# nihalsid/retrieval-fuse

Measured on AMD Instinct MI355X. Metric: 64^3 TSDF chunks/sec (retrieve+attend+refine), higher is better.
Workload: dtype f32

## Files before the change

### include/rfuse.h

```cpp
#ifndef RFUSE_H
#define RFUSE_H

#include <stdint.h>
#include <stddef.h>

#ifdef __cplusplus
extern "C" {
#endif

#define RF_OK 0
#define RF_E_INVALID (-1)
#define RF_E_UNSUPPORTED (-2)
#define RF_E_LAUNCH (-3)
#define RF_E_WORKSPACE (-4)

int rf_abi_version(void);
const char* rf_last_error(void);


int rf_conv3_pack_weight(const float* w_oidhw, int cout, int cin, float* w_packed, void* stream);
size_t rf_conv3_packed_floats(int cout, int cin);

int rf_gn_stats(const float* src0, int c0, const float* src1, int c1, int n, int edge,
                const float* gamma, const float* beta, int groups, float eps,
                float* gn_affine, void* ws, size_t ws_bytes, void* stream);
size_t rf_gn_stats_ws_bytes(int n, int groups);

int rf_conv3d_k3_gn_relu(const float* src0, int c0, const float* src1, int c1, int n, int edge,
                         const float* gn_affine, const float* w_packed, int cout,
                         float* out, void* stream);

int rf_conv3d_k3_gn_relu_stats(const float* src0, int c0, const float* src1, int c1, int n, int edge,
                               const float* gn_affine, const float* w_packed, int cout,
                               float* out, double* stats, void* stream);
int rf_conv3d_stats_tiles(int c0, int c1, int n, int edge, int cout);

int rf_gn_from_stats(const double* stats0, int c0, int tiles0, const double* stats1, int c1, int tiles1, int n, int edge,
                     const float* gamma, const float* beta, int groups, float eps, float* gn_affine, void* stream);

int rf_conv3d_k3_gn_relu_direct(const float* src0, int c0, const float* src1, int c1, int n, int edge,
                                const float* gn_affine, const float* w_oidhw, int cout,
                                float* out, void* stream);

int rf_maxpool3d_2(const float* x, int n, int c, int edge, float* out, void* stream);
int rf_maxpool3d_2_stats(const float* x, int n, int c, int edge, float* out, double* stats, void* stream);
int rf_maxpool_stats_tiles(int edge);

int rf_conv1x1_tanh(const float* x, int n, int c, size_t voxels, const float* w, const float* b,
                    float post_add, float post_mul, float* out, void* stream);

int rf_conv3d_valid_leaky(const float* x, int n, int cin, int s, const float* w, const float* bias, int cout, int k,
                          int stride, float slope, float* out, void* stream);

int rf_conv3d_valid_leaky_mfma(const float* x, int n, int cin, int s, const float* w_packed, const float* bias, int cout, int k,
                               int stride, float slope, float* out, void* stream);
int rf_convv_pack_weight(const float* w_oidhw, int cout, int cin, int k, float* w_packed, void* stream);
size_t rf_convv_packed_floats(int cout, int cin, int k);

int rf_conv3d_valid_lds_supported(int n, int cin, int s, int cout, int k, int stride);
int rf_conv3d_valid_leaky_lds(const float* x, int n, int cin, int s, const float* w_packed, const float* bias, int cout, int k,
                              int stride, float slope, float* out, void* stream);
int rf_convv_lds_pack_weight(const float* w_oidhw, int cout, int cin, int k, float* w_packed, void* stream);
size_t rf_convv_lds_packed_floats(int cout, int cin, int k);

int rf_conv3d_valid_split_supported(int n, int cin, int s, int cout, int k, int stride);
int rf_conv3d_valid_leaky_split(const float* x, int n, int cin, int s, const void* w_packed, const float* bias, int cout, int k,
                                int stride, float slope, float* out, void* stream);
int rf_conv3d_valid_leaky_split_ex(const void* x, int in_split, int n, int cin, int s, const void* w_packed, const float* bias, int cout, int k,
                                   int stride, float slope, void* out, int out_split, void* stream);
int rf_convv_split_pack_weight(const float* w_oidhw, int cout, int cin, int k, int s, int stride, void* w_packed, void* stream);
size_t rf_convv_split_packed_bytes(int cout, int cin, int k, int s, int stride);
int rf_conv3d_valid_split_pg_supported(int n, int cin, int s, int cout, int k, int stride);
int rf_conv3d_valid_leaky_split_pg(const void* x, int n, int cin, int s, const void* w_packed, const float* bias, int cout, int k, int stride,
                                   float slope, void* out, void* stream);
int rf_convv_split_pg_pack_weight(const float* w_oidhw, int cout, int cin, int k, int s, int stride, void* w_packed, void* stream);
size_t rf_convv_split_pg_packed_bytes(int cout, int cin, int k, int s, int stride);

int rf_conv3d_valid_valu_supported(int n, int cin, int s, int cout, int k, int stride);
int rf_conv3d_valid_leaky_valu(const float* x, int n, int cin, int s, const float* w_t, const float* bias, int cout, int k,
                               int stride, float slope, float* out, void* stream);
int rf_conv3d_valid_leaky_valu_ex(const float* x, int n, int cin, int s, const float* w_t, const float* bias, int cout, int k,
                                  int stride, float slope, void* out, int out_split, void* stream);

int rf_conv3d_pool_supported(int c0, int c1, int n, int edge, int cout);
int rf_conv3d_k3_gn_relu_pool(const float* src0, int c0, const float* src1, int c1, int n, int edge,
                              const float* gn_affine, const float* w_packed, int cout,
                              float* out, double* stats, float* pool_out, double* pool_stats, void* stream);

size_t rf_conv3_up_packed_floats(int cout, int c0, int c1);
int rf_conv3_up_pack_weight(const float* w_oidhw, int cout, int c0, int c1, float* w_packed, void* stream);
int rf_conv3d_up_supported(int c0, int c1, int n, int edge, int cout);
int rf_conv3d_up_stats_tiles(int c0, int c1, int n, int edge, int cout);
int rf_conv3d_up_variant(int c0, int c1, int n, int edge, int cout);
int rf_conv3d_up_k3_gn_relu(const float* src0, int c0, const float* src1, int c1, int n, int edge,
                            const float* gn_affine, const float* w_packed, int cout, float* out, double* stats, void* stream);

size_t rf_conv3_up_split_packed_bytes(int cout, int c0, int c1);
int rf_conv3_up_split_pack_weight(const float* w_oidhw, int cout, int c0, int c1, void* w_packed, void* stream);
int rf_conv3d_up_split_supported(int c0, int c1, int n, int edge, int cout);
int rf_conv3d_up_split_stats_tiles(int c0, int c1, int n, int edge, int cout);
int rf_conv3d_up_split_k3_gn_relu(const float* src0, int c0, const float* src1, int c1, int n, int edge,
                                  const float* gn_affine, const void* w_packed, int cout, float* out, double* stats, void* stream);

size_t rf_conv3_split_packed_bytes(int cout, int cin);
int rf_conv3_split_pack_weight(const float* w_oidhw, int cout, int cin, void* w_packed, void* stream);
int rf_conv3d_split_supported(int c0, int c1, int n, int edge, int cout);
int rf_conv3d_split_k3_gn_relu(const float* src, int cin, int n, int edge, const float* gn_affine, const void* w_packed, int cout,
                               float* out, double* stats, float* pool_out, double* pool_stats, void* stream);

size_t rf_conv3_e2_split_packed_bytes(int cout, int cin, int edge);
int rf_conv3_e2_split_pack_weight(const float* w_oidhw, int cout, int cin, int edge, void* w_packed, void* stream);
int rf_conv3d_e2_split_supported(int cin, int n, int edge, int cout);
int rf_conv3d_e2_split_k3_gn_relu(const float* src, int cin, int n, int edge, const float* gn_affine, const void* w_packed, int cout,
                                  float* out, double* stats, void* stream);

size_t rf_split_act_bytes(int n, int c, int edge);
int rf_conv3d_cin1_presplit_supported(int n, int edge, int cout, int next_groups);
int rf_conv3d_cin1_presplit(const float* src, int n, int edge, const float* in_gamma, const float* in_beta, float in_eps, const float* w_packed, int cout,
                            const float* next_gamma, const float* next_beta, int next_groups, float eps, void* out_presplit, void* stream);

int rf_conv3d_split_pointwise_supported(int cin, int n, int edge, int cout);
int rf_conv3d_split_k3_gn_relu_pointwise_tanh(const float* src, int cin, int n, int edge, const float* gn_affine, const void* w_packed, int cout,
                                              const float* pw_w, const float* pw_b, float post_add, float post_mul, float* out1, void* stream);

int rf_conv3d_split_presplit_supported(int cin, int n, int edge, int cout, int next_groups);
int rf_conv3d_split_presplit(const float* src, int cin, int n, int edge, const float* gn_affine, const void* w_packed, int cout, const float* next_gamma,
                             const float* next_beta, int next_groups, float eps, void* out_presplit, double* stats, void* stream);
int rf_conv3d_up_split_presplit_supported(int c0, int c1, int n, int edge, int cout, int next_groups);
int rf_conv3d_up_split_presplit(const float* src0, int c0, const float* src1, int c1, int n, int edge, const float* gn_affine, const void* w_packed,
                                int cout, const float* next_gamma, const float* next_beta, int next_groups, float eps, void* out_presplit,
                                double* stats, void* stream);
int rf_conv3d_split_pre_supported(int cin, int n, int edge, int cout);
int rf_conv3d_split_pre_stats_tiles(int cin, int n, int edge, int cout);
int rf_conv3d_split_pre_k3_relu(const void* src_presplit, int cin, int n, int edge, const void* w_packed, int cout,
                                float* out, double* stats, float* pool_out, double* pool_stats, void* stream);
int rf_conv3d_up_split_presplit_pm_supported(int c0, int c1, int n, int edge, int cout, int next_groups);
int rf_conv3d_up_split_presplit_pm(const float* src0, int c0, const float* src1, int c1, int n, int edge, const float* gn_affine, const void* w_packed,
                                   int cout, const float* next_gamma, const float* next_beta, int next_groups, float eps, void* out_presplit_pm,
                                   double* stats, void* stream);
int rf_conv3d_split_pre_pm_supported(int cin, int n, int edge, int cout);
int rf_conv3d_split_pre_pm_k3_relu(const void* src_presplit_pm, int cin, int n, int edge, const void* w_packed, int cout,
                                   float* out, double* stats, float* pool_out, double* pool_stats, void* stream);


int rf_conv3d_k3_gn(const float* src0, int c0, const float* src1, int c1, int n, int edge,
                    const float* gn_affine, const float* w_packed, int cout, int relu, float* out, void* stream);
int rf_relu_backward(const float* dy, const float* y, size_t count, float* out, void* stream);
int rf_relu_backward_amax_slots(void);
int rf_relu_backward_amax(const float* dy, const float* y, size_t count, float* out, float* amax_slots, void* stream);
int rf_dgrad_scale_affine(const float* amax_slots, int rows, float* affine, float* scales, void* stream);
int rf_conv3d_split_k3_gn_supported(int cin, int n, int edge, int cout);
int rf_conv3d_split_k3_gn(const float* src, int cin, int n, int edge, const float* gn_affine, const void* w_packed, int cout, int relu,
                          float* out, void* stream);
int rf_maxpool3d_2_backward(const float* x, const float* dy, int n, int c, int edge, float* dx, void* stream);
int rf_upsample3d_2(const float* lo, int n, int c, int edge_lo, float* hi, void* stream);
int rf_sumpool3d_2(const float* hi, int n, int c, int edge, float* lo, void* stream);
int rf_gn_backward(const float* x, const float* dxn, int n, int c, int edge, const float* gamma, int groups, float eps, const float* dxn_inv_scale,
                   float* dx, float* dgamma, float* dbeta, void* ws, size_t ws_bytes, void* stream);
size_t rf_gn_backward_ws_bytes(int n, int c, int edge);
int rf_conv3d_k3_wgrad(const float* x, int cin, int n, int edge, const float* gn_affine, const float* dz, int cout, float* dw, void* ws,
                       size_t ws_bytes, void* stream);
size_t rf_conv3d_k3_wgrad_ws_bytes(int cin, int cout, int n, int edge);
int rf_conv3d_k3_wgrad_split_supported(int cin, int cout, int n, int edge);
size_t rf_conv3d_k3_wgrad_split_ws_bytes(int cin, int cout, int n, int edge);
int rf_conv3d_k3_wgrad_split(const float* x, int cin, int n, int edge, const float* gn_affine, const float* dz, int cout, const float* scales,
                             float* dw, void* ws, size_t ws_bytes, void* stream);

size_t rf_conv3d_valid_leaky_backward_ws_bytes(int n, int cout, int so);
int rf_conv3d_valid_leaky_backward(const float* dy, const float* y, int n, int cout, int so, float slope, float* dz, float* db, void* ws,
                                   size_t ws_bytes, void* stream);
size_t rf_convv_dgrad_packed_floats(int cout, int cin, int k);
int rf_conv3d_valid_dgrad(const float* dz, int n, int cout, int so, const float* wd_packed, int cin, int k, int stride, int s, float* dx, void* stream);
size_t rf_conv3d_valid_wgrad_ws_bytes(int n, int cin, int cout, int so, int k);
int rf_conv3d_valid_wgrad(const float* x, int n, int cin, int s, const float* dz, int cout, int k, int stride, float* dw, void* ws, size_t ws_bytes,
                          void* stream);


int rf_unfold3d(const float* x, int b, int c, int s, int e, float* rows, void* stream);
int rf_fold3d(const float* rows, int b, int c, int s, int e, float* x, void* stream);


int rf_linear_pack_weight(const float* w, int nout, int nin, float* w_packed, void* stream);
size_t rf_linear_packed_floats(int nout, int nin);

#define RF_ACT_NONE 0
#define RF_ACT_RELU 1
#define RF_ACT_LEAKY 2
int rf_linear(const float* x, int rows, int nin, const float* w_packed, const float* bias, int nout,
              int act, float slope, float* y, void* stream);

int rf_linear_wgrad(const float* a, const float* b, int K, int M, int N, float* dw, void* ws, size_t ws_bytes, void* stream);
size_t rf_linear_wgrad_ws_bytes(int K, int M, int N);

int rf_l2_normalize_rows(float* x, int rows, int dim, float eps, void* stream);


#define RF_ATTN_SOFTMAX 0
#define RF_ATTN_GUMBEL_HARD 1
int rf_attn_fuse(const float* x, const float* p, const float* xf, const float* pf, const float* noise,
                 int b, int k, int d, int f, int mode, float sharpness,
                 float* out, float* scores_out, float* weights_out, void* stream);

int rf_attn_gather_retrieved(const float* src, int src_layout, int b, int k, int c, int s, int e, int t,
                             float* p_rows, void* stream);

size_t rf_attn_mlp_split_packed_floats(int n_in);
int rf_attn_mlp_split_pack(const float* w1, const float* w2, const float* w3, const float* w4, int n_in, float* packed_split, void* stream);
int rf_attn_mlp_split_rows(const float* x, int rows, int n_in, const float* packed, const float* packed_split, float* out, void* stream);
int rf_attn_mlp_split_volume(const float* src, int b, int kv, int c, int s, int t, const float* packed, const float* packed_split,
                             float* out, void* stream);
size_t rf_attn_mlp_packed_floats(int n_in);
int rf_attn_mlp_pack(const float* w1, const float* b1, const float* w2, const float* b2, const float* w3, const float* b3,
                     const float* w4, const float* b4, int n_in, float* packed, void* stream);
int rf_attn_mlp_rows(const float* x, int rows, int n_in, const float* packed, float* out, void* stream);
int rf_attn_mlp_volume(const float* src, int b, int kv, int c, int s, int t, const float* packed, float* out, void* stream);
int rf_attn_weights(const float* xf, const float* pf, const float* noise, int rows, int k, int f, int mode, float sharpness,
                    float* weights, float* switches, float* scores_out, void* stream);
int rf_attn_weights_sampled(const float* xf, const float* pf, int rows, int k, int f, float sharpness, void* rng_state,
                            float* weights, float* switches, float* scores_out, float* noise_out, void* stream);
int rf_attn_blend(const float* x, const float* retrieved, int b, int k, int c, int s, int t, const float* weights,
                  const float* switches, float* out, void* stream);


int rf_query_windows(const float* raw, int b, int s, int ps, int ctx, float pad_value, float mean, float stddev,
                     float* out, void* stream);

int rf_gather_windows(const float* grid, int n, int c, int g, int w, int step, int np, float* out, void* stream);
int rf_gather_windows_split(const void* grid, int n, int c, int g, int w, int step, int np, void* out, void* stream);

int rf_db_pack_embeddings(const float* emb, int64_t n, int dim, float* packed, void* stream);
size_t rf_db_packed_floats(int64_t n, int dim);

int rf_l2_topk(const float* q, int nq, int dim, const float* db_packed, int64_t n, int64_t row_base, int k2, int algo,
               float* out_dist, int64_t* out_idx, void* ws, size_t ws_bytes, void* stream);
size_t rf_l2_topk_ws_bytes(int nq, int64_t n, int k2);
int rf_l2_topk_keys(const float* q, int nq, int dim, const float* db_packed, int64_t n, int64_t row_base, int k2, int algo,
                    uint64_t* out_keys, void* ws, size_t ws_bytes, void* stream);
int rf_topk_merge_keys(const uint64_t* in_keys, int parts, int nq, int k2, float* out_dist, int64_t* out_idx, void* stream);

int rf_topk_merge(const float* in_dist, const int64_t* in_idx, int parts, int nq, int k2,
                  float* out_dist, int64_t* out_idx, void* stream);

int rf_demote_same_scene(const float* dist, const int64_t* idx, int nq, int k2, const int32_t* db_meta,
                         const int32_t* query_scene, const uint8_t* query_keep, int K, int32_t* out_meta, float* out_dist,
                         int64_t* out_idx, void* stream);

int rf_gather_patches(const float* db_volumes, int64_t n_scenes, const int32_t* meta, int chunks, int K,
                      float trunc_fill, float trunc_ratio, float mean, float stddev, int layout,
                      float* out, void* stream);

int rf_gather_patches_f16(const void* db_volumes_f16, int64_t n_scenes, const int32_t* meta, int chunks, int K,
                          float trunc_fill, float trunc_ratio, float mean, float stddev, int layout,
                          float* out, void* stream);
int rf_compose_overlap(const void* db_volumes, int half, int64_t n_scenes, const float* mapping, const int32_t* boxes, int P, int K, int sx, int sy, int sz,
                       float trunc_fill, float trunc_ratio, float* out, float* dist_ws, void* stream);

int rf_gather_rows(const float* src, int64_t n_src, const int64_t* idx, int64_t m, int width, float* out, void* stream);


size_t rf_conv3d_split_pre_pool_presplit_scratch_floats(int cout);
int rf_conv3d_split_pre_pool_presplit_supported(int cin, int n, int edge, int cout, int next_groups);
int rf_conv3d_split_pre_k3_relu_pool_presplit(const void* src_presplit, int cin, int n, int edge, const void* w_packed, int cout, float* pool_scratch,
                                              double* pool_stats, const float* next_gamma, const float* next_beta, int next_groups, float eps,
                                              void* out_presplit, void* stream);
int rf_conv3d_split_pre_presplit_supported(int cin, int n, int edge, int cout, int next_groups);
int rf_conv3d_split_pre_presplit(const void* src_presplit, int cin, int n, int edge, const void* w_packed, int cout, const float* next_gamma,
                                 const float* next_beta, int next_groups, float eps, void* out_presplit, double* stats, void* stream);
// ... 30 lines not shown
```

### retrieval-fuse_amd/csrc/conv3d_e2_split.hip

```cpp
#include "common.h"
#include "split_operand.h"

namespace {
constexpr int E2_NC = 256;
constexpr int E2_STEP_H8 = (E2_NC / 16) * 2 * 64;
constexpr int E2_LDS_BYTES = 2 * E2_STEP_H8 * 16;
}

__host__ __device__ static inline size_t e2_chunks(int cout, int edge) { return ((size_t)cout * (edge == 2 ? 8 : 1) + E2_NC - 1) / E2_NC; }
__host__ __device__ static inline size_t e2_ksteps(int cin, int edge) { return edge == 2 ? (size_t)(cin + 3) / 4 : (size_t)(cin + 31) / 32; }

extern "C" size_t rf_conv3_e2_split_packed_bytes(int cout, int cin, int edge) {
    return e2_chunks(cout, edge) * e2_ksteps(cin, edge) * E2_STEP_H8 * 16;
}

__global__ void k_conv3_e2_split_pack(const float* __restrict__ w, int cout, int cin, int edge, h8* __restrict__ wp, size_t total) {
    const int ksteps = (int)e2_ksteps(cin, edge);
    for (size_t i = (size_t)blockIdx.x * blockDim.x + threadIdx.x; i < total; i += (size_t)gridDim.x * blockDim.x) {
        const int lane = (int)(i & 63), piece = (int)((i >> 6) & 1), t = (int)((i >> 7) & 15);
        const size_t st = i >> 11;
        const int s = (int)(st % ksteps), chunk = (int)(st / ksteps);
        const int col = chunk * E2_NC + t * 16 + (lane & 15);
        h8 out;
#pragma unroll
// ... 8 lines not shown
            } else {
                const int co = col, ci = 32 * s + 8 * (lane >> 4) + u;
                if (co < cout && ci < cin) val = (double)w[((size_t)co * cin + ci) * 27 + 13];
            }
            _Float16 h, l;
            rf_split_weight(val, h, l);
            out[u] = piece == 0 ? h : l;
        }
        wp[i] = out;
    }
}

extern "C" int rf_conv3_e2_split_pack_weight(const float* w_oidhw, int cout, int cin, int edge, void* w_packed, void* stream) {
    RF_REQUIRE(w_oidhw && w_packed && cout > 0 && cin > 0 && (edge == 1 || edge == 2), RF_E_INVALID, "rf_conv3_e2_split_pack_weight: bad arguments");
    const size_t total = rf_conv3_e2_split_packed_bytes(cout, cin, edge) / 16;
    return rf_launch<k_conv3_e2_split_pack>("rf_conv3_e2_split_pack_weight", dim3(rf_blocks(total, 256, 4096)), dim3(256), (hipStream_t)stream, w_oidhw, cout, cin, edge,
                                            reinterpret_cast<h8*>(w_packed), total);
}

struct E2Args {
    const float* src;
    const float4* affine;
    const h8* wp;
    float* out;
    double2* stats;
    int cin, cout, n;
};

template <int V, int MT>
__global__ __launch_bounds__(256, 2) void k_conv3_e2_split(E2Args a) {
    constexpr int WN = MT == 64 ? 2 : 4, NJ = 16 / WN;
    extern __shared__ __attribute__((aligned(16))) unsigned char lds_raw[];
    h8* bufs = reinterpret_cast<h8*>(lds_raw);
    const int tid = threadIdx.x, lane = tid & 63;
    const int wave = __builtin_amdgcn_readfirstlane(tid >> 6);
    const int wm = MT == 64 ? wave >> 1 : 0, wn = MT == 64 ? wave & 1 : wave;
    const int li = lane & 15, kg = lane >> 4;
    const int n0 = blockIdx.x * MT, chunk = blockIdx.y;
    const int cin = a.cin, cout = a.cout, ksteps = V == 8 ? cin >> 2 : (cin + 31) >> 5;
    const h8* __restrict__ wsrc = a.wp + (size_t)chunk * ksteps * E2_STEP_H8 + tid;

    const float* xrow[2];
    const float4* arow[2];
#pragma unroll
    for (int i = 0; i < 2; ++i) {
        int sm = n0 + (2 * wm + i) * 16 + li;
        sm = sm < a.n ? sm : a.n - 1;
        xrow[i] = a.src + (V == 8 ? ((size_t)sm * cin + kg) * 8 : (size_t)sm * cin + kg * 8);
        arow[i] = a.affine + (V == 8 ? (size_t)sm * cin + kg : (size_t)sm * cin + kg * 8);
    }
    f32x4 hi[2][NJ], lo[2][NJ];
#pragma unroll
    for (int i = 0; i < 2; ++i)
#pragma unroll
        for (int j = 0; j < NJ; ++j) { hi[i][j] = f32x4{0.f, 0.f, 0.f, 0.f}; lo[i][j] = f32x4{0.f, 0.f, 0.f, 0.f}; }

    float4 xa[2][2], af[2];
    h8 nah[2], nal[2];
    h8 wreg[8];
    auto split1 = [](float y, _Float16& hh, _Float16& ll) { rf_split(y * SPLIT_ACT_SCALE, hh, ll); };
    auto load_step = [&](int s) {
#pragma unroll
        for (int i = 0; i < 2; ++i) {
            if constexpr (V == 8) {
                xa[i][0] = *reinterpret_cast<const float4*>(xrow[i] + (size_t)s * 32);
                xa[i][1] = *reinterpret_cast<const float4*>(xrow[i] + (size_t)s * 32 + 4);
                af[i] = arow[i][(size_t)s * 4];
            } else {
#pragma unroll
                for (int j = 0; j < 8; ++j) {
                    const bool ok = 32 * s + 8 * kg + j < cin;
                    const float x = ok ? xrow[i][(size_t)s * 32 + j] : 0.f;
                    const float4 t = ok ? arow[i][(size_t)s * 32 + j] : make_float4(0.f, 0.f, 0.f, 0.f);
                    _Float16 hh, ll;
                    split1(fmaf(x - t.x, t.y, t.z), hh, ll);
                    nah[i][j] = hh; nal[i][j] = ll;
                }
            }
        }
#pragma unroll
        for (int q = 0; q < 8; ++q) wreg[q] = wsrc[(size_t)s * E2_STEP_H8 + q * 256];
    };
    auto store_b = [&](int buf) {
#pragma unroll
        for (int q = 0; q < 8; ++q) bufs[buf * E2_STEP_H8 + q * 256 + tid] = wreg[q];
    };
    load_step(0);
    store_b(0);
    h8 ah[2], al[2];
    auto convert = [&] {
#pragma unroll
        for (int i = 0; i < 2; ++i) {
            if constexpr (V == 8) {
                const float raw[8] = {xa[i][0].x, xa[i][0].y, xa[i][0].z, xa[i][0].w, xa[i][1].x, xa[i][1].y, xa[i][1].z, xa[i][1].w};
#pragma unroll
                for (int j = 0; j < 8; ++j) {
                    _Float16 hh, ll;
                    split1(fmaf(raw[j] - af[i].x, af[i].y, af[i].z), hh, ll);
                    ah[i][j] = hh; al[i][j] = ll;
                }
            } else {
                ah[i] = nah[i]; al[i] = nal[i];
            }
        }
    };
    convert();
    __syncthreads();

    for (int s = 0; s < ksteps; ++s) {
        const bool more = s + 1 < ksteps;
        if (more) load_step(s + 1);
        const h8* bb = bufs + (s & 1) * E2_STEP_H8 + (wn * NJ) * 128 + lane;
#pragma unroll
        for (int j = 0; j < NJ; ++j) {
            const h8 bh = bb[j * 128], bl = bb[j * 128 + 64];
#pragma unroll
            for (int i = 0; i < 2; ++i) {
                hi[i][j] = __builtin_amdgcn_mfma_f32_16x16x32_f16(ah[i], bh, hi[i][j], 0, 0, 0);
                lo[i][j] = __builtin_amdgcn_mfma_f32_16x16x32_f16(ah[i], bl, lo[i][j], 0, 0, 0);
                lo[i][j] = __builtin_amdgcn_mfma_f32_16x16x32_f16(al[i], bh, lo[i][j], 0, 0, 0);
            }
        }
        if (more) {
            store_b((s + 1) & 1);
            convert();
        }
        __syncthreads();
    }

    const int ncols = cout * V;
#pragma unroll
    for (int i = 0; i < 2; ++i)
#pragma unroll
        for (int j = 0; j < NJ; ++j) {
            const int col = chunk * E2_NC + (wn * NJ + j) * 16 + li;
#pragma unroll
            for (int r = 0; r < 4; ++r) {
                const int sm = n0 + (2 * wm + i) * 16 + kg * 4 + r;
                const float y = rf_relu(rf_split_join(hi[i][j][r], lo[i][j][r]));
                const bool live = sm < a.n && col < ncols;
                if (live) a.out[(size_t)sm * ncols + col] = y;
                if (a.stats) {
                    double sv = (double)y, sq = (double)y * (double)y;
                    if constexpr (V == 8) {
#pragma unroll
                        for (int d = 1; d <= 4; d <<= 1) { sv += __shfl_xor(sv, d, 64); sq += __shfl_xor(sq, d, 64); }
                    }
                    if (live && (V == 1 || (li & 7) == 0)) a.stats[(size_t)sm * cout + (V == 8 ? col >> 3 : col)] = make_double2(sv, sq);
                }
            }
        }
}

extern "C" int rf_conv3d_e2_split_supported(int cin, int n, int edge, int cout) {
    if (edge == 1) return cin >= 8 && cout >= 2 && n >= 16;
    return edge == 2 && cin >= 8 && cin % 4 == 0 && cout >= 2 && n >= 16;
}

extern "C" int rf_conv3d_e2_split_k3_gn_relu(const float* src, int cin, int n, int edge, const float* gn_affine, const void* w_packed, int cout,
                                              float* out, double* stats, void* stream) {
    RF_REQUIRE(rf_conv3d_e2_split_supported(cin, n, edge, cout), RF_E_UNSUPPORTED,
               "rf_conv3d_e2_split_k3_gn_relu: takes whole 2^3 volumes (cin a multiple of 4) or 1^3 volumes, cin >= 8, at least 16 samples (got cin=%d n=%d edge=%d cout=%d)", cin, n, edge, cout);
    RF_REQUIRE(src && gn_affine && w_packed && out, RF_E_INVALID, "rf_conv3d_e2_split_k3_gn_relu: null pointer");
    E2Args a;
    a.src = src; a.affine = reinterpret_cast<const float4*>(gn_affine); a.wp = reinterpret_cast<const h8*>(w_packed); a.out = out;
    a.stats = reinterpret_cast<double2*>(stats); a.cin = cin; a.cout = cout; a.n = n;
    const unsigned chunks = (unsigned)e2_chunks(cout, edge);
    const bool wide = (long long)((n + 63) / 64) * chunks >= rf_persistent_wgs() / RF_PERSIST_ROUNDS;
    const dim3 grid((unsigned)((n + (wide ? 63 : 31)) / (wide ? 64 : 32)), chunks);
    const char* who = "rf_conv3d_e2_split_k3_gn_relu";
    hipStream_t s = (hipStream_t)stream;
    if (edge == 2)
        return wide ? rf_launch<k_conv3_e2_split<8, 64>>(who, grid, dim3(256), E2_LDS_BYTES, E2_LDS_BYTES, s, a)
                    : rf_launch<k_conv3_e2_split<8, 32>>(who, grid, dim3(256), E2_LDS_BYTES, E2_LDS_BYTES, s, a);
    return wide ? rf_launch<k_conv3_e2_split<1, 64>>(who, grid, dim3(256), E2_LDS_BYTES, E2_LDS_BYTES, s, a)
                : rf_launch<k_conv3_e2_split<1, 32>>(who, grid, dim3(256), E2_LDS_BYTES, E2_LDS_BYTES, s, a);
}
```

### retrieval-fuse_amd/rfuse/ops.py

```python
import ctypes
import functools
import sys
import weakref

import torch

from . import _lib

ACT_NONE, ACT_RELU, ACT_LEAKY = 0, 1, 2
ATTN_SOFTMAX, ATTN_GUMBEL_HARD = 0, 1


def _req(t, name, dtype=torch.float32):
    if not isinstance(t, torch.Tensor):
        raise TypeError('%s: expected a torch.Tensor' % name)
    if not t.is_cuda:
        raise RuntimeError('%s: the refinement hot path runs on the GPU only (got a %s tensor); there is no CPU fallback' % (name, t.device))
    if t.dtype != dtype:
        raise TypeError('%s: expected %s, got %s' % (name, dtype, t.dtype))
    if not t.is_contiguous():
        raise ValueError('%s: tensor must be contiguous' % name)
    return t


# ... 177 lines not shown
        lib.rf_conv3d_k3_gn_relu(_p(src0), c0, _p(src1), c1, n, edge, _p(aff), _p(w_packed), cout, _p(out),
                                 _stream())


def conv3d_gn_relu(src0, src1, aff, w_packed, cout, direct_weight=None):
    n, c0, c1, edge = _src_dims(src0, src1)
    dev = _check_affine(aff, n, c0 + c1)
    out = torch.empty((n, cout, edge, edge, edge), dtype=torch.float32, device=dev)
    lib = _lib.load()
    if direct_weight is not None:
        lib.rf_conv3d_k3_gn_relu_direct(_p(src0), c0, _p(src1), c1, n, edge, _p(aff), _p(direct_weight.detach()),
                                        cout, _p(out), _stream())
    else:
        _conv_launch(lib, src0, c0, src1, c1, n, edge, aff, w_packed, cout, out)
    return out


USE_FUSED_POOL = True


def conv_pool_supported(src0, src1, cout):
    if not USE_FUSED_POOL:
        return False
    n, c0, c1, edge = _src_dims(src0, src1)
    return bool(_lib.load().rf_conv3d_pool_supported(c0, c1, n, edge, cout))


def conv3d_gn_relu_pool(src0, src1, aff, w_packed, cout, keep_full=True):
    n, c0, c1, edge = _src_dims(src0, src1)
    dev = _check_affine(aff, n, c0 + c1)
    lib = _lib.load()
    out = torch.empty((n, cout, edge, edge, edge), dtype=torch.float32, device=dev) if keep_full else None
    pooled = torch.empty((n, cout, edge // 2, edge // 2, edge // 2), dtype=torch.float32, device=dev)
    tiles = lib.rf_conv3d_stats_tiles(c0, c1, n, edge, cout)
    pstats = _attach_stats(pooled, tiles)
    lib.rf_conv3d_k3_gn_relu_pool(_p(src0), c0, _p(src1), c1, n, edge, _p(aff), _p(w_packed), cout, _p(out), _p(_attach_stats(out, tiles)),
                                  _p(pooled), _p(pstats), _stream())
    return out, pooled


def pack_conv3_up_weight(w, c0):
    _req(w.detach(), 'conv weight')
    cout, cin = w.shape[0], w.shape[1]
    if tuple(w.shape[2:]) != (3, 3, 3) or not 0 <= c0 < cin:
        raise ValueError('pack_conv3_up_weight: expected an OIDHW 3x3x3 weight and 0 <= c0 < cin, got %s, c0=%d' % (tuple(w.shape), c0))
    return _pack_weight('conv3_up', w, (cout, c0, cin - c0))


def conv_up_supported(src0, src1, cout):
    if src1 is None or not USE_CONV_UP:
        return False
    n, c0, c1, edge = _src_dims(src0, src1)
    return bool(_lib.load().rf_conv3d_up_supported(c0, c1, n, edge, cout))


USE_CONV_UP = True


def conv3d_up_gn_relu(src0, src1, aff, w_up_packed, cout):
    n, c0, c1, edge = _src_dims(src0, src1)
    out = torch.empty((n, cout, edge, edge, edge), dtype=torch.float32, device=_check_affine(aff, n, c0 + c1))
    lib = _lib.load()
    stats = _attach_stats(out, lib.rf_conv3d_up_stats_tiles(c0, c1, n, edge, cout))
    lib.rf_conv3d_up_k3_gn_relu(_p(src0), c0, _p(src1), c1, n, edge, _p(aff), _p(w_up_packed), cout, _p(out),
                                _p(stats), _stream())
    return out


CONV_ARITH = 'split'

SPLIT_MAX_ABS_WEIGHT = 65504.0 / 16 / 8
SPLIT_MAX_ABS_ACT = 65504.0 * 16
_range_cache = {}
_range_seen = weakref.WeakValueDictionary()


def _range_key(t):
    return (t.data_ptr(), tuple(t.shape), t.device)


def _abs_max(t):
    key = _range_key(t)
    hit = _range_cache.get(key)
    if hit is not None and hit[0] == t._version:
        return hit[1]
    if t.is_cuda and torch.cuda.is_current_stream_capturing():
        raise RuntimeError('range check of a parameter inside a graph capture: run one step before capturing (RefinementEngine.capture_graph does)')
    if len(_range_cache) > 8192:
        _range_cache.clear()
    _range_seen[id(t)] = t
    stale = [u for u in list(_range_seen.values())
             if u.device == t.device and u.dtype == t.dtype and u.numel() > 0 and _range_cache.get(_range_key(u), (None,))[0] != u._version]
    if t.is_cuda and len(stale) > 1:
        vals = torch.stack(torch._foreach_norm([u.detach() for u in stale], float('inf'))).tolist()
        for u, val in zip(stale, vals):
            _range_cache[_range_key(u)] = (u._version, float(val))
        return _range_cache[key][1]
    v = float(t.detach().abs().max().item())
    _range_cache[key] = (t._version, v)
    return v


def split_range_ok(weight, gamma=None, beta=None, group_elements=0):
    w_ok = _abs_max(weight) <= SPLIT_MAX_ABS_WEIGHT
    if gamma is None:
        return w_ok
    return w_ok and _abs_max(gamma) * (float(group_elements) ** 0.5) + _abs_max(beta) <= SPLIT_MAX_ABS_ACT


def pack_conv3_split_weight(w):
    _req(w.detach(), 'conv weight')
    if tuple(w.shape[2:]) != (3, 3, 3):
        raise ValueError('pack_conv3_split_weight: expected an OIDHW 3x3x3 weight, got %s' % (tuple(w.shape),))
    return _pack_weight('conv3_split', w, (w.shape[0], w.shape[1]), torch.uint8)


def conv_split_supported(src0, src1, cout):
    if src1 is not None or src0 is None or CONV_ARITH != 'split':
        return False
    n, c0, c1, edge = _src_dims(src0, src1)
    return bool(_lib.load().rf_conv3d_split_supported(c0, c1, n, edge, cout))


def conv3d_split_gn_relu(src, aff, w_split_packed, cout, pool=None):
    n, cin, _, edge = _src_dims(src, None)
    if edge == 4 and pool is not None:
        out = conv3d_split_gn_relu(src, aff, w_split_packed, cout)
        return (out if pool == 'also' else None), maxpool2(out)
    dev = _check_affine(aff, n, cin)
    lib = _lib.load()
    out = torch.empty((n, cout, edge, edge, edge), dtype=torch.float32, device=dev) if pool != 'only' else None
    pooled = torch.empty((n, cout, edge // 2, edge // 2, edge // 2), dtype=torch.float32, device=dev) if pool is not None else None
    tiles = max(1, (edge // 8) ** 3)
    stats, pstats = _attach_stats(out, tiles), _attach_stats(pooled, tiles)
    lib.rf_conv3d_split_k3_gn_relu(_p(src), cin, n, edge, _p(aff), _p(w_split_packed), cout, _p(out), _p(stats), _p(pooled), _p(pstats),
                                   _stream())
    return out if pool is None else (out, pooled)


def pack_conv3_e2_split_weight(w, edge=2):
    _req(w.detach(), 'conv weight')
    if tuple(w.shape[2:]) != (3, 3, 3) or edge not in (1, 2):
        raise ValueError('pack_conv3_e2_split_weight: expected an OIDHW 3x3x3 weight and edge 1 or 2, got %s, edge %r' % (tuple(w.shape), edge))
    return _pack_weight('conv3_e2_split', w, (w.shape[0], w.shape[1], edge), torch.uint8)


def conv_e2_split_supported(src, cout):
    if src is None or CONV_ARITH != 'split':
        return False
    n, c0, _, edge = _src_dims(src, None)
    return bool(_lib.load().rf_conv3d_e2_split_supported(c0, n, edge, cout))


def conv3d_e2_split_gn_relu(src, aff, w_e2_packed, cout):
    n, cin, _, edge = _src_dims(src, None)
    dev = _check_affine(aff, n, cin)
    out = torch.empty((n, cout, edge, edge, edge), dtype=torch.float32, device=dev)
    _lib.load().rf_conv3d_e2_split_k3_gn_relu(_p(src), cin, n, edge, _p(aff), _p(w_e2_packed), cout, _p(out), _p(_attach_stats(out, 1)), _stream())
    return out


USE_PRESPLIT = True


def cin1_presplit_supported(x, cout, next_groups, next_cout):
    if not USE_PRESPLIT or CONV_ARITH != 'split' or x is None or x.shape[1] != 1:
        return False
    n, edge = x.shape[0], x.shape[2]
    lib = _lib.load()
    return bool(lib.rf_conv3d_cin1_presplit_supported(n, edge, cout, next_groups)) and bool(lib.rf_conv3d_split_pre_supported(cout, n, edge, next_cout))


def conv3d_cin1_presplit(x, in_gamma, in_beta, in_eps, w_packed, cout, next_gamma, next_beta, next_groups, eps):
    _req(x, 'x')
    n, edge = x.shape[0], x.shape[2]
    lib = _lib.load()
    out = torch.empty(lib.rf_split_act_bytes(n, cout, edge), dtype=torch.uint8, device=x.device)
    lib.rf_conv3d_cin1_presplit(_p(x), n, edge, _p(in_gamma.detach()), _p(in_beta.detach()), in_eps, _p(w_packed), cout, _p(next_gamma.detach()),
                                _p(next_beta.detach()), next_groups, eps, _p(out), _stream())
    return out


def conv_split_pointwise_supported(x, cout):
    return CONV_ARITH == 'split' and x is not None and bool(_lib.load().rf_conv3d_split_pointwise_supported(x.shape[1], x.shape[0], x.shape[2], cout))


def conv3d_split_pointwise_tanh(x, gn_affine_t, w_split_packed, cout, pw_w, pw_b, post_add=0.0, post_mul=1.0):
    _req(x, 'x')
    n, cin, edge = x.shape[0], x.shape[1], x.shape[2]
    if pw_w.shape[0] != 1:
        raise NotImplementedError('conv3d_split_pointwise_tanh: one output channel (Conv3d(nf,1,1), model/refinement.py:54)')
    out = torch.empty((n, 1, edge, edge, edge), dtype=torch.float32, device=x.device)
    _lib.load().rf_conv3d_split_k3_gn_relu_pointwise_tanh(_p(x), cin, n, edge, _p(gn_affine_t), _p(w_split_packed), cout, _p(pw_w.detach()), _p(pw_b.detach()),
                                                          post_add, post_mul, _p(out), _stream())
    return out


def conv_split_presplit_supported(x, cout, next_groups):
    return (USE_PRESPLIT and CONV_ARITH == 'split' and x is not None
            and bool(_lib.load().rf_conv3d_split_presplit_supported(x.shape[1], x.shape[0], x.shape[2], cout, next_groups)))


def conv3d_split_presplit(x, gn_affine_t, w_split_packed, cout, next_gamma, next_beta, next_groups, eps):
    _req(x, 'x')
    n, cin, edge = x.shape[0], x.shape[1], x.shape[2]
    lib = _lib.load()
    out = torch.empty(lib.rf_split_act_bytes(n, cout, edge), dtype=torch.uint8, device=x.device)
    lib.rf_conv3d_split_presplit(_p(x), cin, n, edge, _p(gn_affine_t), _p(w_split_packed), cout, _p(next_gamma.detach()), _p(next_beta.detach()),
                                 next_groups, eps, _p(out), _p(None), _stream())
    return out


def conv_up_split_presplit_supported(x, upsampled, cout, next_groups):
    if not USE_PRESPLIT or CONV_ARITH != 'split' or upsampled is None:
        return False
    c0 = x.shape[1] if x is not None else 0
    return bool(_lib.load().rf_conv3d_up_split_presplit_supported(c0, upsampled.shape[1], upsampled.shape[0], 2 * upsampled.shape[2], cout, next_groups))


def conv_up_split_presplit_pm_supported(x, upsampled, cout, next_groups, next_cout):
    if not USE_PRESPLIT or CONV_ARITH != 'split' or upsampled is None or x is None:
        return False
    lib = _lib.load()
    n, edge = upsampled.shape[0], 2 * upsampled.shape[2]
    return bool(lib.rf_conv3d_up_split_presplit_pm_supported(x.shape[1], upsampled.shape[1], n, edge, cout, next_groups)) and \
        bool(lib.rf_conv3d_split_pre_pm_supported(cout, n, edge, next_cout))


def conv3d_up_split_presplit(x, upsampled, gn_affine_t, w_packed, cout, next_gamma, next_beta, next_groups, eps, parity_major=False):
    _req(upsampled, 'upsampled')
    n, edge = upsampled.shape[0], 2 * upsampled.shape[2]
    c0 = x.shape[1] if x is not None else 0
    lib = _lib.load()
    out = torch.empty(lib.rf_split_act_bytes(n, cout, edge), dtype=torch.uint8, device=upsampled.device)
    c1 = upsampled.shape[1]
    launch = lib.rf_conv3d_up_split_presplit_pm if parity_major else lib.rf_conv3d_up_split_presplit
    launch(_p(x), c0, _p(upsampled), c1, n, edge, _p(gn_affine_t), _p(w_packed), cout, _p(next_gamma.detach()),
           _p(next_beta.detach()), next_groups, eps, _p(out), _p(None), _stream())
    return out


USE_PREPOOL = True


class PreSplit:

    def __init__(self, data, n, channels, edge):
        self.data, self.n, self.channels, self.edge = data, n, channels, edge

    @property
    def device(self):
        return self.data.device


def conv_split_supported_shape(n, cin, edge, cout):
    return CONV_ARITH == 'split' and bool(_lib.load().rf_conv3d_split_supported(int(cin), 0, int(n), int(edge), int(cout)))


def conv_split_pre_pool_presplit_supported(cin, n, edge, cout, next_groups):
    return USE_PREPOOL and USE_PRESPLIT and CONV_ARITH == 'split' and bool(_lib.load().rf_conv3d_split_pre_pool_presplit_supported(cin, n, edge, cout, next_groups))


def conv3d_split_pre_relu_pool_presplit(pre, cin, n, edge, w_split_packed, cout, next_gamma, next_beta, next_groups, eps):
    dev = pre.device
    lib = _lib.load()
    half = edge // 2
    scratch = torch.empty(lib.rf_conv3d_split_pre_pool_presplit_scratch_floats(cout), dtype=torch.float32, device=dev)
    out = torch.empty(lib.rf_split_act_bytes(n, cout, half), dtype=torch.uint8, device=dev)
    lib.rf_conv3d_split_pre_k3_relu_pool_presplit(_p(pre), cin, n, edge, _p(w_split_packed), cout, _p(scratch), _p(None), _p(next_gamma.detach()),
                                                  _p(next_beta.detach()), next_groups, eps, _p(out), _stream())
    return None, PreSplit(out, n, cout, half)


def conv_split_pre_presplit_supported(cin, n, edge, cout, next_groups):
    return USE_PRESPLIT and CONV_ARITH == 'split' and bool(_lib.load().rf_conv3d_split_pre_presplit_supported(cin, n, edge, cout, next_groups))


def conv3d_split_pre_presplit(pre, w_split_packed, cout, next_gamma, next_beta, next_groups, eps):
    lib = _lib.load()
    out = torch.empty(lib.rf_split_act_bytes(pre.n, cout, pre.edge), dtype=torch.uint8, device=pre.device)
    lib.rf_conv3d_split_pre_presplit(_p(pre.data), pre.channels, pre.n, pre.edge, _p(w_split_packed), cout, _p(next_gamma.detach()), _p(next_beta.detach()),
                                     next_groups, eps, _p(out), _p(None), _stream())
    return PreSplit(out, pre.n, cout, pre.edge)


def conv3d_split_pre_relu(pre, cin, n, edge, w_split_packed, cout, pool=None, parity_major=False):
    dev = pre.device
    lib = _lib.load()
    out = torch.empty((n, cout, edge, edge, edge), dtype=torch.float32, device=dev) if pool != 'only' else None
    pooled = torch.empty((n, cout, edge // 2, edge // 2, edge // 2), dtype=torch.float32, device=dev) if pool is not None else None
    tiles = 1 if parity_major else lib.rf_conv3d_split_pre_stats_tiles(cin, n, edge, cout)
    stats, pstats = _attach_stats(out, tiles), _attach_stats(pooled, tiles)
    launch = lib.rf_conv3d_split_pre_pm_k3_relu if parity_major else lib.rf_conv3d_split_pre_k3_relu
    launch(_p(pre), cin, n, edge, _p(w_split_packed), cout, _p(out), _p(stats), _p(pooled), _p(pstats), _stream())
    if pool is None:
        return out
    return out, pooled


def conv_split_issued_flops(cin, n, edge, cout):
    return 2.0 * 3 * -(-cin // 8) * 7 * 32 * (-(-cout // 16) * 16) * edge ** 3 * n


def pack_conv3_up_split_weight(w, c0):
    _req(w.detach(), 'conv weight')
    cout, cin = w.shape[0], w.shape[1]
    if tuple(w.shape[2:]) != (3, 3, 3) or not 0 <= c0 < cin:
        raise ValueError('pack_conv3_up_split_weight: expected an OIDHW 3x3x3 weight and 0 <= c0 < cin, got %s, c0=%d' % (tuple(w.shape), c0))
    return _pack_weight('conv3_up_split', w, (cout, c0, cin - c0), torch.uint8)


# ... 617 lines not shown
```

Baseline: 5009.

## Add weight-stationary LDS kernel for 2^3 split conv with planner selecting form

```diff
diff --git a/include/rfuse.h b/include/rfuse.h
--- a/include/rfuse.h
+++ b/include/rfuse.h
@@ -113,6 +113,9 @@
 int rf_conv3d_e2_split_supported(int cin, int n, int edge, int cout);
 int rf_conv3d_e2_split_k3_gn_relu(const float* src, int cin, int n, int edge, const float* gn_affine, const void* w_packed, int cout,
                                   float* out, double* stats, void* stream);
+size_t rf_conv3d_e2_split_plan(int cin, int n, int edge, int cout, int cus, int* form, int* cols, int* groups);
+int64_t rf_conv3d_e2_split_k3_gn_relu_form(const float* src, int cin, int n, int edge, const float* gn_affine, const void* w_packed, int cout,
+                                           float* out, double* stats, void* stream, int form);
 
 size_t rf_split_act_bytes(int n, int c, int edge);
 int rf_conv3d_cin1_presplit_supported(int n, int edge, int cout, int next_groups);
diff --git a/retrieval-fuse_amd/csrc/conv3d_e2_split.hip b/retrieval-fuse_amd/csrc/conv3d_e2_split.hip
--- a/retrieval-fuse_amd/csrc/conv3d_e2_split.hip
+++ b/retrieval-fuse_amd/csrc/conv3d_e2_split.hip
@@ -184,27 +184,265 @@
         }
 }
 
+namespace {
+constexpr int E2S_WAVES = 8;
+constexpr int E2S_LDS_MAX = 128 * 1024;
+typedef float f32x3 __attribute__((ext_vector_type(3)));
+typedef int i32x4 __attribute__((ext_vector_type(4)));
+}
+
+template <int V, int NJ>
+__global__ __launch_bounds__(E2S_WAVES * 64) void k_conv3_e2_split_ws(E2Args a, int nbs, int ppg) {
+    constexpr int D = V == 8 ? 4 : 1;
+    extern __shared__ __attribute__((aligned(16))) unsigned char lds_raw[];
+    h8* wl = reinterpret_cast<h8*>(lds_raw);
+    const int tid = threadIdx.x, lane = tid & 63;
+    const int wave = __builtin_amdgcn_readfirstlane(tid >> 6);
+    const int li = lane & 15, kg = lane >> 4;
+    const int from_lane = 4 * (4 * li + kg);
+    const int cin = a.cin, cout = a.cout, ksteps = V == 8 ? cin >> 2 : (cin + 31) >> 5;
+    const int t0 = blockIdx.y * nbs;
+    const int njg = nbs / NJ, nitems = ppg * njg;
+
+    const float* xrow[2];
+    const float4* arow[2];
+    float4 xa[D][2][2];
+    f32x3 af[D][2];
+    float x1[D][2][8], t1[D][2][8][3];
+    int m0 = 0, jn = 0;
+    auto split1 = [](float y, _Float16& hh, _Float16& ll) { rf_split(y * SPLIT_ACT_SCALE, hh, ll); };
+    auto load_a = [&](int d, int s) {
+#pragma unroll
+        for (int i = 0; i < 2; ++i) {
+            if constexpr (V == 8) {
+                xa[d][i][0] = *reinterpret_cast<const float4*>(xrow[i] + (size_t)s * 32);
+                xa[d][i][1] = *reinterpret_cast<const float4*>(xrow[i] + (size_t)s * 32 + 4);
+                af[d][i] = *reinterpret_cast<const f32x3*>(arow[i] + (size_t)s * 4);
+            } else {
+#pragma unroll
+                for (int j = 0; j < 8; ++j) {
+                    const bool ok = 32 * s + 8 * kg + j < cin;
+                    const int off = ok ? s * 32 + j : cin - 1 - 8 * kg;
+                    const float x = xrow[i][off];
+                    const float4 t = arow[i][off];
+                    x1[d][i][j] = ok ? x : 0.f;
+                    t1[d][i][j][0] = ok ? t.x : 0.f; t1[d][i][j][1] = ok ? t.y : 0.f; t1[d][i][j][2] = ok ? t.z : 0.f;
+                }
+            }
+        }
+    };
+    auto begin_item = [&](int item) {
+        m0 = (blockIdx.x * ppg + item / njg) * 32;
+        jn = (item % njg) * NJ;
+        if (item >= nitems || m0 >= a.n) return false;
+#pragma unroll
+        for (int i = 0; i < 2; ++i) {
+            int sm = m0 + i * 16 + (V == 8 ? lane >> 2 : li);
+            sm = sm < a.n ? sm : a.n - 1;
+            xrow[i] = a.src + (V == 8 ? ((size_t)sm * cin + (lane & 3)) * 8 : (size_t)sm * cin + kg * 8);
+            arow[i] = a.affine + (V == 8 ? (size_t)sm * cin + (lane & 3) : (size_t)sm * cin + kg * 8);
+        }
+#pragma unroll
+        for (int d = 0; d < D; ++d) load_a(d, d < ksteps ? d : ksteps - 1);
+        return true;
+    };
+    int item = wave;
+    bool live = begin_item(item);
+
+    {
+        const int shift = 7 + (nbs >> 1), run = 1 << shift, total = ksteps << shift;
+        const h8* __restrict__ wsrc = a.wp + ((size_t)(t0 >> 4) * ksteps * 16 + (t0 & 15)) * 128;
+        for (int base = tid; base < total; base += E2S_WAVES * 64 * 8) {
+            h8 r[8];
+#pragma unroll
+            for (int q = 0; q < 8; ++q) {
+                int i = base + q * E2S_WAVES * 64;
+                i = i < total ? i : total - 1;
+                r[q] = wsrc[(size_t)(i >> shift) * E2_STEP_H8 + (i & (run - 1))];
+            }
+#pragma unroll
+            for (int q = 0; q < 8; ++q) {
+                const int i = base + q * E2S_WAVES * 64;
+                if (i < total) wl[i] = r[q];
+            }
+        }
+    }
+    __syncthreads();
+
+    const int ncols = cout * V;
+    while (live) {
+        f32x4 hi[2][NJ], lo[2][NJ];
+#pragma unroll
+        for (int i = 0; i < 2; ++i)
+#pragma unroll
+            for (int j = 0; j < NJ; ++j) { hi[i][j] = f32x4{0.f, 0.f, 0.f, 0.f}; lo[i][j] = f32x4{0.f, 0.f, 0.f, 0.f}; }
+        const h8* bb = wl + (size_t)jn * 128 + lane;
+        auto step = [&](int d, int s, bool more) {
+            h8 ah[2], al[2];
+#pragma unroll
+            for (int i = 0; i < 2; ++i) {
+                if constexpr (V == 8) {
+                    const float raw[8] = {xa[d][i][0].x, xa[d][i][0].y, xa[d][i][0].z, xa[d][i][0].w, xa[d][i][1].x, xa[d][i][1].y, xa[d][i][1].z, xa[d][i][1].w};
+#pragma unroll
+                    for (int j = 0; j < 8; ++j) {
+                        _Float16 hh, ll;
+                        split1(fmaf(raw[j] - af[d][i][0], af[d][i][1], af[d][i][2]), hh, ll);
+                        ah[i][j] = hh; al[i][j] = ll;
+                    }
+                    i32x4 wh = __builtin_bit_cast(i32x4, ah[i]), wl4 = __builtin_bit_cast(i32x4, al[i]);
+#pragma unroll
+                    for (int q = 0; q < 4; ++q) {
+                        wh[q] = __builtin_amdgcn_ds_bpermute(from_lane, wh[q]);
+                        wl4[q] = __builtin_amdgcn_ds_bpermute(from_lane, wl4[q]);
+                    }
+                    ah[i] = __builtin_bit_cast(h8, wh); al[i] = __builtin_bit_cast(h8, wl4);
+                } else {
+#pragma unroll
+                    for (int j = 0; j < 8; ++j) {
+                        _Float16 hh, ll;
+                        split1(fmaf(x1[d][i][j] - t1[d][i][j][0], t1[d][i][j][1], t1[d][i][j][2]), hh, ll);
+                        ah[i][j] = hh; al[i][j] = ll;
+                    }
+                }
+            }
+            if (more) load_a(d, s + D < ksteps ? s + D : ksteps - 1);
+            const h8* bs = bb + (size_t)s * nbs * 128;
+#pragma unroll
+            for (int j = 0; j < NJ; ++j) {
+                const h8 bh = bs[j * 128], bl = bs[j * 128 + 64];
+                hi[0][j] = __builtin_amdgcn_mfma_f32_16x16x32_f16(ah[0], bh, hi[0][j], 0, 0, 0);
+                lo[0][j] = __builtin_amdgcn_mfma_f32_16x16x32_f16(ah[0], bl, lo[0][j], 0, 0, 0);
+                hi[1][j] = __builtin_amdgcn_mfma_f32_16x16x32_f16(ah[1], bh, hi[1][j], 0, 0, 0);
+                lo[1][j] = __builtin_amdgcn_mfma_f32_16x16x32_f16(ah[1], bl, lo[1][j], 0, 0, 0);
+                lo[0][j] = __builtin_amdgcn_mfma_f32_16x16x32_f16(al[0], bh, lo[0][j], 0, 0, 0);
+                lo[1][j] = __builtin_amdgcn_mfma_f32_16x16x32_f16(al[1], bh, lo[1][j], 0, 0, 0);
+            }
+            __builtin_amdgcn_sched_barrier(0);
+        };
+        int s0 = 0;
+        for (; s0 + D <= ksteps; s0 += D) {
+#pragma unroll
+            for (int d = 0; d < D; ++d) step(d, s0 + d, true);
+        }
+#pragma unroll
+        for (int d = 0; d < D - 1; ++d)
+            if (s0 + d < ksteps) step(d, s0 + d, false);
+        const int em0 = m0, ejn = jn;
+        item += E2S_WAVES;
+        live = begin_item(item);
+
+#pragma unroll
+        for (int i = 0; i < 2; ++i)
+#pragma unroll
+            for (int j = 0; j < NJ; ++j) {
+                const int col = (t0 + ejn + j) * 16 + li;
+#pragma unroll
+                for (int r = 0; r < 4; ++r) {
+                    const int sm = em0 + i * 16 + kg * 4 + r;
+                    const float y = rf_relu(rf_split_join(hi[i][j][r], lo[i][j][r]));
+                    const bool ok = sm < a.n && col < ncols;
+                    if (ok) a.out[(size_t)sm * ncols + col] = y;
+                    if (a.stats) {
+                        double sv = (double)y, sq = (double)y * (double)y;
+                        if constexpr (V == 8) {
+#pragma unroll
+                            for (int d = 1; d <= 4; d <<= 1) { sv += __shfl_xor(sv, d, 64); sq += __shfl_xor(sq, d, 64); }
+                        }
+                        if (ok && (V == 1 || (li & 7) == 0)) a.stats[(size_t)sm * cout + (V == 8 ? col >> 3 : col)] = make_double2(sv, sq);
+                    }
+                }
+            }
+    }
+}
+
 extern "C" int rf_conv3d_e2_split_supported(int cin, int n, int edge, int cout) {
     if (edge == 1) return cin >= 8 && cout >= 2 && n >= 16;
     return edge == 2 && cin >= 8 && cin % 4 == 0 && cout >= 2 && n >= 16;
 }
 
-extern "C" int rf_conv3d_e2_split_k3_gn_relu(const float* src, int cin, int n, int edge, const float* gn_affine, const void* w_packed, int cout,
-                                              float* out, double* stats, void* stream) {
+struct E2SPlan { int cols, slices, groups, ppg, lds; };
+static bool e2s_plan(int cin, int n, int edge, int cout, int cus, E2SPlan& p) {
+    const long long ncols = (long long)cout * (edge == 2 ? 8 : 1), ksteps = (long long)e2_ksteps(cin, edge);
+    int c = 64;
+    while (c >= 16 && ksteps * (c / 16) * 2048 > E2S_LDS_MAX) c >>= 1;
+    if (c < 16) return false;
+    while (c > 16 && c / 2 >= ncols) c >>= 1;
+    const long long slices = (ncols + c - 1) / c;
+    const int pairs = (n + 31) / 32;
+    const long long want = cus / slices < 1 ? 1 : (cus / slices < pairs ? cus / slices : pairs);
+    p.cols = c; p.slices = (int)slices; p.ppg = (int)((pairs + want - 1) / want); p.groups = (pairs + p.ppg - 1) / p.ppg; p.lds = (int)(ksteps * (c / 16) * 2048);
+    return true;
+}
+
+static bool e2_stream_wide(int n, int edge, int cout, int cus) { return (long long)((n + 63) / 64) * (long long)e2_chunks(cout, edge) >= 2LL * cus; }
+static int e2_stream_groups(int n, int edge, int cout, int cus) { return e2_stream_wide(n, edge, cout, cus) ? (n + 63) / 64 : (n + 31) / 32; }
+static bool e2_stationary(int cin, int n, int edge, int cout, int cus, E2SPlan& p) {
+    if (edge != 2 || !e2s_plan(cin, n, edge, cout, cus, p) || p.slices > 2LL * cus) return false;
+    const double chunks = (double)e2_chunks(cout, edge), wgs = e2_stream_groups(n, edge, cout, cus) * chunks;
+    if (wgs < cus) return true;
+    const double samples = 6.0 * n * 8 * cin;
+    return p.slices * samples + (double)p.slices * p.groups * p.lds <= chunks * samples + wgs * (double)e2_ksteps(cin, edge) * (E2_STEP_H8 * 16);
+}
+
+extern "C" size_t rf_conv3d_e2_split_plan(int cin, int n, int edge, int cout, int cus, int* form, int* cols, int* groups) {
+    RF_REQUIRE(form && cols && groups && cus > 0, 0, "rf_conv3d_e2_split_plan: bad arguments");
+    RF_REQUIRE(rf_conv3d_e2_split_supported(cin, n, edge, cout), 0, "rf_conv3d_e2_split_plan: not a layer of the 2^3 / 1^3 GEMM form (cin=%d n=%d edge=%d cout=%d)", cin, n, edge, cout);
+    E2SPlan p;
+    if (e2_stationary(cin, n, edge, cout, cus, p)) {
+        *form = 2; *cols = p.cols; *groups = p.groups;
+        return (size_t)p.lds;
+    }
+    *form = 1; *cols = E2_NC; *groups = e2_stream_groups(n, edge, cout, cus);
+    return E2_LDS_BYTES;
+}
+
+extern "C" int64_t rf_conv3d_e2_split_k3_gn_relu_form(const float* src, int cin, int n, int edge, const float* gn_affine, const void* w_packed, int cout,
+                                                   float* out, double* stats, void* stream, int form) {
+    const char* who = "rf_conv3d_e2_split_k3_gn_relu";
     RF_REQUIRE(rf_conv3d_e2_split_supported(cin, n, edge, cout), RF_E_UNSUPPORTED,
                "rf_conv3d_e2_split_k3_gn_relu: takes whole 2^3 volumes (cin a multiple of 4) or 1^3 volumes, cin >= 8, at least 16 samples (got cin=%d n=%d edge=%d cout=%d)", cin, n, edge, cout);
     RF_REQUIRE(src && gn_affine && w_packed && out, RF_E_INVALID, "rf_conv3d_e2_split_k3_gn_relu: null pointer");
+    RF_REQUIRE(form >= 0 && form <= 2, RF_E_INVALID, "rf_conv3d_e2_split_k3_gn_relu: form is 0 (auto), 1 (streaming) or 2 (weight-stationary), got %d", form);
     E2Args a;
     a.src = src; a.affine = reinterpret_cast<const float4*>(gn_affine); a.wp = reinterpret_cast<const h8*>(w_packed); a.out = out;
     a.stats = reinterpret_cast<double2*>(stats); a.cin = cin; a.cout = cout; a.n = n;
+    const int cus = rf_resident_wgs() / 2;
+    E2SPlan p;
+    const bool stationary = form == 0 && e2_stationary(cin, n, edge, cout, cus, p);
+    const bool fits = form == 2 && e2s_plan(cin, n, edge, cout, cus, p);
+    RF_REQUIRE(form != 2 || fits, RF_E_UNSUPPORTED, "rf_conv3d_e2_split_k3_gn_relu: the weight-stationary form cannot hold a 16-column slice of K = %d in %d bytes of LDS",
+               (int)e2_ksteps(cin, edge) * 32, E2S_LDS_MAX);
+    hipStream_t s = (hipStream_t)stream;
+    if (form == 2 || stationary) {
+        const int nbs = p.cols / 16, ppg = p.ppg, lds = p.lds;
+        const dim3 grid((unsigned)p.groups, (unsigned)p.slices);
+        const dim3 block(E2S_WAVES * 64);
+        const int nj = ppg >= E2S_WAVES ? nbs : 1;
+        int rc;
+        if (edge == 2) {
+            if (nj == 4) rc = rf_launch<k_conv3_e2_split_ws<8, 4>>(who, grid, block, (size_t)lds, E2S_LDS_MAX, s, a, nbs, ppg);
+            else if (nj == 2) rc = rf_launch<k_conv3_e2_split_ws<8, 2>>(who, grid, block, (size_t)lds, E2S_LDS_MAX, s, a, nbs, ppg);
+            else rc = rf_launch<k_conv3_e2_split_ws<8, 1>>(who, grid, block, (size_t)lds, E2S_LDS_MAX, s, a, nbs, ppg);
+        }
+        else if (nj >= 2) rc = rf_launch<k_conv3_e2_split_ws<1, 2>>(who, grid, block, (size_t)lds, E2S_LDS_MAX, s, a, nbs, ppg);
+        else rc = rf_launch<k_conv3_e2_split_ws<1, 1>>(who, grid, block, (size_t)lds, E2S_LDS_MAX, s, a, nbs, ppg);
+        return rc ? rc : 2;
+    }
     const unsigned chunks = (unsigned)e2_chunks(cout, edge);
-    const bool wide = (long long)((n + 63) / 64) * chunks >= rf_persistent_wgs() / RF_PERSIST_ROUNDS;
-    const dim3 grid((unsigned)((n + (wide ? 63 : 31)) / (wide ? 64 : 32)), chunks);
-    const char* who = "rf_conv3d_e2_split_k3_gn_relu";
-    hipStream_t s = (hipStream_t)stream;
+    const dim3 grid((unsigned)e2_stream_groups(n, edge, cout, cus), chunks);
+    const bool wide = e2_stream_wide(n, edge, cout, cus);
+    int rc;
     if (edge == 2)
-        return wide ? rf_launch<k_conv3_e2_split<8, 64>>(who, grid, dim3(256), E2_LDS_BYTES, E2_LDS_BYTES, s, a)
-                    : rf_launch<k_conv3_e2_split<8, 32>>(who, grid, dim3(256), E2_LDS_BYTES, E2_LDS_BYTES, s, a);
-    return wide ? rf_launch<k_conv3_e2_split<1, 64>>(who, grid, dim3(256), E2_LDS_BYTES, E2_LDS_BYTES, s, a)
-                : rf_launch<k_conv3_e2_split<1, 32>>(who, grid, dim3(256), E2_LDS_BYTES, E2_LDS_BYTES, s, a);
-}
+        rc = wide ? rf_launch<k_conv3_e2_split<8, 64>>(who, grid, dim3(256), E2_LDS_BYTES, E2_LDS_BYTES, s, a)
+                  : rf_launch<k_conv3_e2_split<8, 32>>(who, grid, dim3(256), E2_LDS_BYTES, E2_LDS_BYTES, s, a);
+    else
+        rc = wide ? rf_launch<k_conv3_e2_split<1, 64>>(who, grid, dim3(256), E2_LDS_BYTES, E2_LDS_BYTES, s, a)
+                  : rf_launch<k_conv3_e2_split<1, 32>>(who, grid, dim3(256), E2_LDS_BYTES, E2_LDS_BYTES, s, a);
+    return rc ? rc : 1;
+}
+
+extern "C" int rf_conv3d_e2_split_k3_gn_relu(const float* src, int cin, int n, int edge, const float* gn_affine, const void* w_packed, int cout,
+                                              float* out, double* stats, void* stream) {
+    const int64_t rc = rf_conv3d_e2_split_k3_gn_relu_form(src, cin, n, edge, gn_affine, w_packed, cout, out, stats, stream, 0);
+    return rc < 0 ? (int)rc : RF_OK;
+}
diff --git a/retrieval-fuse_amd/rfuse/ops.py b/retrieval-fuse_amd/rfuse/ops.py
--- a/retrieval-fuse_amd/rfuse/ops.py
+++ b/retrieval-fuse_amd/rfuse/ops.py
@@ -353,11 +353,17 @@
     return bool(_lib.load().rf_conv3d_e2_split_supported(c0, n, edge, cout))
 
 
-def conv3d_e2_split_gn_relu(src, aff, w_e2_packed, cout):
+def conv3d_e2_split_gn_relu(src, aff, w_e2_packed, cout, form=0):
     n, cin, _, edge = _src_dims(src, None)
     dev = _check_affine(aff, n, cin)
     out = torch.empty((n, cout, edge, edge, edge), dtype=torch.float32, device=dev)
-    _lib.load().rf_conv3d_e2_split_k3_gn_relu(_p(src), cin, n, edge, _p(aff), _p(w_e2_packed), cout, _p(out), _p(_attach_stats(out, 1)), _stream())
+    if form:
+        rc = _lib.load().rf_conv3d_e2_split_k3_gn_relu_form(_p(src), cin, n, edge, _p(aff), _p(w_e2_packed), cout, _p(out), _p(_attach_stats(out, 1)), _stream(), int(form))
+        if rc < 0:
+            _lib.check(rc, 'rf_conv3d_e2_split_k3_gn_relu_form')
+        out._rf_e2_form = rc
+    else:
+        _lib.load().rf_conv3d_e2_split_k3_gn_relu(_p(src), cin, n, edge, _p(aff), _p(w_e2_packed), cout, _p(out), _p(_attach_stats(out, 1)), _stream())
     return out
 
 
```

Result: no change. 5003 (-0.1%).
